# isgasho/h2o-kubernetes

Measured on AMD Instinct MI355X. Metric: GBM train rows/sec on HIGGS-shape 11M×28 at 1/2/4/8 MI355X; AUC parity, higher is better.
Workload: dtype fp32 gradients/hessians; histograms in fixed-point int32 (stochastic rounding) summed exactly in int64; fp64 split gains; exact int64 leaf sums; uint8 bins; 1 GPU; model=GBM bernoulli, global_batch=11000000, rows_per_gpu=11000000, cols=28, max_depth=5, nbins=255, parallelism=dp1

## Files before the change

### h2omx/csrc/tree_kernels.hip

```cpp
#include "common.h"
#include "p2p_device.h"
#include <math.h>

#include <algorithm>
#include <cstdlib>

namespace {

struct SplitParams {
  int mode;
  int leaf_mode;
  int F;
  int is_last_level;
  double min_rows;
  double min_child_weight;
  double lambda_;
  double alpha;
  double gamma;
  double min_split_improvement;
  double learn_rate;
  double max_abs_leaf;
  uint32_t seed;
  int tree_index;
  int depth;
// ... 643 lines not shown
      if (2 * ks > lv.max_next_nodes) ks = lv.max_next_nodes / 2;
      *res_s = ks;
    }
  }
  __syncthreads();
  return *res_s;
}

struct LevelFin {
  LevelOut lv;
  int* ticket;
};

template <int MODE>
__device__ void level_fin_records(const FeatBest* __restrict__ fbest, const int* __restrict__ ctl, const SplitParams& p,
                                  int nbt, const LevelOut& lv) {
  const int n = ctl[CTL_N];
  const int lane = threadIdx.x & 63, wid = threadIdx.x >> 6, nw = blockDim.x >> 6;
  for (int node = wid; node < n; node += nw) node_best_wave<MODE>(fbest, p.F, node, lane, lv.nsplit);
  __syncthreads();
  level_finalize_body(ctl, p, nbt, lv);
}

constexpr int CMP_STAGE_BYTES = 2048;
constexpr int HB_PF = 1;

template <int NBT, int ROWS, int PKM, bool ROUTE, bool CMP, int COP = 1, bool NID16 = false>
__global__ __launch_bounds__(1024) void hist_build_kernel(
    const uint8_t* __restrict__ codes, int64_t npad, const float* __restrict__ g, const float* __restrict__ s2,
    const int* __restrict__ nid, const NodeLink* __restrict__ link, const int* __restrict__ ctl,
    const int* __restrict__ nvb, const double* __restrict__ qscale, uint32_t salt, int F, int fg, int n_groups,
    int wgpg, int slot_lo, int slot_cnt, const short* __restrict__ slot16, unsigned long long* __restrict__ pk_buf,
    unsigned long long* __restrict__ partials, const PartInfo* __restrict__ part_prev,
    const int* __restrict__ ctl_prev, int* __restrict__ nid_out, int writer, GradFuse gf, LevelPro lp,
    const uint8_t* __restrict__ joint, const int* __restrict__ plane_src) {
  salt = (uint32_t)qscale[9];
  extern __shared__ __attribute__((aligned(16))) unsigned long long lds64[];
  __shared__ int width_s[256], rep_s[256];
  __shared__ float rcp_s[256];
  __shared__ NodeSplit pro_ns[ROUTE ? PRO_MAX_NODES : 1];
  __shared__ PartInfo pro_ps[ROUTE ? PRO_MAX_NODES : 1];
  __shared__ int pro_res;
  bool pro = false;
  if constexpr (ROUTE) pro = lp.fbest != nullptr;
  int n_slots;
  if (pro) n_slots = level_prologue(lp, ctl_prev, NBT, blockIdx.x == 0 && writer != 0, pro_ns, pro_ps, &pro_res);
  else n_slots = ctl[CTL_SLOTS];
  const int b = blockIdx.x;
  const int xcd = b & 7, i = b >> 3;
  const int group = i % n_groups;
  const int chunk = xcd + 8 * (i / n_groups);
  const bool route_w = ROUTE && writer && group == 0 && ctl_prev[CTL_N] > 0;
  const bool build = slot_lo < n_slots;
  if (!build && !route_w) return;
  const int f0 = group * fg;
  const int nf = min(fg, F - f0);
  static_assert(COP == 1 || ((PKM == 1 || PKM == 3 || PKM == 6) && !ROUTE && !CMP), "copies: level-0 kernel only");
  const int hist_elems = slot_cnt * fg * NBT;
// ... 2 lines not shown
    const int sp = plane_src ? plane_src[f0 + fi] : f0 + fi;
    return sp >= 0 ? codes + (int64_t)sp * npad : joint + (int64_t)(~sp) * npad;
  };

  for (int j = threadIdx.x; j < hist_elems * COP; j += blockDim.x) lds64[j] = 0ull;
  if (threadIdx.x < fg) {
    const int fi = threadIdx.x;
    const int w = (fi < nf) ? nvb[f0 + fi] + 1 : NBT;
    width_s[fi] = w;
    int r = NBT / w;
    r = r < 1 ? 1 : (r > 64 ? 64 : r);
    if (COP > 1) r = 1;
    rep_s[fi] = r;
    rcp_s[fi] = 1.0f / (float)r;
  }
  __shared__ float tval_s[PKM == 5 ? GF_LDS_NODES : 1];
  if constexpr (PKM == 5) {
    if (gf.apply && gf.cap <= GF_LDS_NODES)
      for (int j = threadIdx.x; j < gf.cap; j += blockDim.x) tval_s[j] = gf.tree[j].value;
  }
  const float sg = (float)qscale[0], ss = (float)qscale[1];
  const int64_t rb = (int64_t)qscale[7];
  const int64_t n_rows = (int64_t)qscale[8];
  __syncthreads();

  const int64_t units = npad / ROWS;
  const int64_t u0 = units * chunk / wgpg, u1 = units * (chunk + 1) / wgpg;
  const int64_t ustart = CMP ? u0 + (threadIdx.x & ~63) : u0 + threadIdx.x;
  for (int64_t uu = ustart; uu < u1; uu += blockDim.x) {
    const bool inb = !CMP || uu + lane < u1;
    const int64_t u = CMP ? (inb ? uu + lane : u1 - 1) : uu;
    const int64_t r0 = u * ROWS;
    int s[ROWS];
    bool any = false;
    if constexpr (ROUTE) {
      int nn[ROWS], nx[ROWS];
      if (nid == nullptr) {
#pragma unroll
        for (int k = 0; k < ROWS; ++k) nn[k] = (r0 + k < n_rows) ? 0 : INT32_MIN;
      } else if constexpr (NID16) {
        const short* n16 = reinterpret_cast<const short*>(nid);
#pragma unroll
        for (int q = 0; q < ROWS / 8; ++q) {
          const uint4 v = *reinterpret_cast<const uint4*>(n16 + r0 + 8 * q);
          const uint32_t w4[4] = {v.x, v.y, v.z, v.w};
#pragma unroll
          for (int k = 0; k < 8; ++k) nn[8 * q + k] = (int)(short)(w4[k >> 1] >> (16 * (k & 1)));
        }
      } else {
#pragma unroll
        for (int q = 0; q < ROWS / 4; ++q) {
          const int4 n4 = *reinterpret_cast<const int4*>(nid + r0 + 4 * q);
          nn[4 * q] = n4.x; nn[4 * q + 1] = n4.y; nn[4 * q + 2] = n4.z; nn[4 * q + 3] = n4.w;
        }
      }
#pragma unroll
      for (int k = 0; k < ROWS; ++k) { nx[k] = nn[k]; s[k] = -1; }
      const int n_prev = pro ? min(ctl_prev[CTL_N], PRO_MAX_NODES) : ctl_prev[CTL_N];
      for (int j = 0; j < n_prev; ++j) {
        bool mine = false;
#pragma unroll
        for (int k = 0; k < ROWS; ++k) mine |= (nn[k] == j);
        if (!mine) continue;
        const PartInfo pj = pro ? pro_ps[j] : part_prev[j];
        if (pj.child < 0) {
#pragma unroll
          for (int k = 0; k < ROWS; ++k)
            if (nn[k] == j) nx[k] = ~pj.gid;
          continue;
        }
        uint32_t cw[ROWS / 4];
        const uint8_t* cp = codes + (int64_t)pj.feat * npad + r0;
        if constexpr (ROWS == 16) {
          const uint4 c4 = *reinterpret_cast<const uint4*>(cp);
          cw[0] = c4.x; cw[1] = c4.y; cw[2] = c4.z; cw[3] = c4.w;
        } else {
          const uint2 c2 = *reinterpret_cast<const uint2*>(cp);
          cw[0] = c2.x; cw[1] = c2.y;
        }
        const int sl_l = (int)(short)(pj.pad & 0xFFFF), sl_r = pj.pad >> 16;
#pragma unroll
        for (int k = 0; k < ROWS; ++k) {
          if (nn[k] == j) {
            const int bc = (cw[k >> 2] >> (8 * (k & 3))) & 0xff;
            const int right = part_right(pj, bc, NBT);
            nx[k] = pj.child + right;
            s[k] = right ? sl_r : sl_l;
          }
        }
      }
#pragma unroll
      for (int k = 0; k < ROWS; ++k) {
        int sl = s[k] - slot_lo;
        if (sl < 0 || sl >= slot_cnt || !build) sl = -1;
        s[k] = sl;
        any |= (sl >= 0);
      }
      if (route_w) {
        if constexpr (NID16) {
          short* o16 = reinterpret_cast<short*>(nid_out);
#pragma unroll
// ... 1074 lines not shown

constexpr int PART_LDS_NODES = 256;

__device__ __forceinline__ int leaf_reps(const double* __restrict__ qs) {
  const int r = (int)qs[10];
  return r < 1 ? 1 : r;
}
constexpr int LEAF_REPS_MAX = 16;
__device__ __forceinline__ long long leaf_sum(const unsigned long long* __restrict__ acc, int64_t i, int reps,
                                              int64_t stride) {
  unsigned long long x[LEAF_REPS_MAX];
#pragma unroll
  for (int r = 0; r < LEAF_REPS_MAX; ++r) x[r] = r < reps ? acc[i + r * stride] : 0ull;
  long long v = 0;
#pragma unroll
  for (int r = 0; r < LEAF_REPS_MAX; ++r) v += (long long)x[r];
  for (int r = LEAF_REPS_MAX; r < reps; ++r) v += (long long)acc[i + r * stride];
  return v;
}
__device__ __forceinline__ void leaf_zero(unsigned long long* __restrict__ acc, int64_t i, int reps, int64_t stride) {
  for (int r = 0; r < reps; ++r) acc[i + r * stride] = 0ull;
}

template <bool PREF, int RPL, int NIDM = 0>
__global__ __launch_bounds__(256) void partition_kernel(const uint8_t* __restrict__ codes, int64_t npad,
                                                        int* nid, const PartInfo* __restrict__ part,
                                                        int nbt, const float* __restrict__ g,
                                                        const float* __restrict__ h, const float* __restrict__ w,
                                                        const double* __restrict__ qs, int cap,
                                                        unsigned long long* __restrict__ leaf_acc,
                                                        const int* __restrict__ ctl_cur,
                                                        const int* __restrict__ ctl_next, int win_max, int R,
                                                        short* __restrict__ slot16, int* nid_out, int all_rows,
                                                        const float* __restrict__ Fm, const float* __restrict__ yv,
                                                        GradParams gp, const uint8_t* __restrict__ y8,
                                                        LevelPro lp) {
  extern __shared__ __attribute__((aligned(16))) unsigned long long lacc[];
  __shared__ PartInfo ps[PART_LDS_NODES];
  __shared__ NodeSplit pro_ns[PRO_MAX_NODES];
  __shared__ int pro_res;
  const bool pro = lp.fbest != nullptr;
  int n_next = 0;
  if (pro) n_next = 2 * level_prologue(lp, ctl_cur, nbt, blockIdx.x == 0, pro_ns, ps, &pro_res);
  const bool use_lds = leaf_acc != nullptr && win_max > 0;
  const int base = all_rows ? 0 : ctl_cur[CTL_BASE];
  const int win = use_lds ? (all_rows ? win_max : min(win_max, ctl_cur[CTL_N] + (pro ? n_next : ctl_next[CTL_N]))) : 0;
  const int n_cur = ctl_cur[CTL_N];
  const bool rec_lds = pro || n_cur <= PART_LDS_NODES;
  if (rec_lds && !pro)
    for (int j = threadIdx.x; j < n_cur; j += blockDim.x) ps[j] = part[j];
  if (use_lds)
    for (int j = threadIdx.x; j < 3 * win * R; j += blockDim.x) lacc[j] = 0ull;
  __syncthreads();
  const int copy = (threadIdx.x & 63) % R;
  float lg = 0, lh = 0, lw = 0;
  if (leaf_acc) { lg = (float)qs[4]; lh = (float)qs[5]; lw = (float)qs[6]; }
  const int64_t nq = npad / RPL;
  for (int64_t q = (int64_t)blockIdx.x * blockDim.x + threadIdx.x; q < nq; q += (int64_t)gridDim.x * blockDim.x) {
    const int64_t r0 = q * RPL;
    int nn[RPL];
    if constexpr (NIDM & 1) {
      static_assert(RPL % 8 == 0, "int16 node ids: 8-row vectors");
#pragma unroll
      for (int v = 0; v < RPL / 8; ++v) {
        const uint4 q4 = *reinterpret_cast<const uint4*>(reinterpret_cast<const short*>(nid) + r0 + 8 * v);
        const uint32_t w4[4] = {q4.x, q4.y, q4.z, q4.w};
#pragma unroll
        for (int k = 0; k < 8; ++k) nn[8 * v + k] = (int)(short)(w4[k >> 1] >> (16 * (k & 1)));
      }
    } else {
#pragma unroll
      for (int v = 0; v < RPL / 4; ++v) {
        const int4 na = *reinterpret_cast<int4*>(nid + r0 + 4 * v);
        nn[4 * v] = na.x; nn[4 * v + 1] = na.y; nn[4 * v + 2] = na.z; nn[4 * v + 3] = na.w;
      }
    }
    float gv[RPL], hv[RPL], wv8[RPL];
    if (PREF) {
#pragma unroll
      for (int v = 0; v < RPL / 4; ++v) {
        if (Fm != nullptr) {
          const float4 f0 = *reinterpret_cast<const float4*>(Fm + r0 + 4 * v);
          float4 y0;
          if (y8 != nullptr) {
            const uint32_t b4 = *reinterpret_cast<const uint32_t*>(y8 + r0 + 4 * v);
            y0 = make_float4((float)(b4 & 0xff), (float)((b4 >> 8) & 0xff), (float)((b4 >> 16) & 0xff),
                             (float)(b4 >> 24));
          } else {
            y0 = *reinterpret_cast<const float4*>(yv + r0 + 4 * v);
          }
          const float fa[4] = {f0.x, f0.y, f0.z, f0.w}, ya[4] = {y0.x, y0.y, y0.z, y0.w};
#pragma unroll
          for (int k = 0; k < 4; ++k) dist_grad(gp.dist, fa[k], ya[k], gp, gv[4 * v + k], hv[4 * v + k]);
        } else {
          const float4 g0 = *reinterpret_cast<const float4*>(g + r0 + 4 * v);
          const float4 h0 = *reinterpret_cast<const float4*>(h + r0 + 4 * v);
          gv[4 * v] = g0.x; gv[4 * v + 1] = g0.y; gv[4 * v + 2] = g0.z; gv[4 * v + 3] = g0.w;
          hv[4 * v] = h0.x; hv[4 * v + 1] = h0.y; hv[4 * v + 2] = h0.z; hv[4 * v + 3] = h0.w;
        }
        if (w) {
          const float4 w0 = *reinterpret_cast<const float4*>(w + r0 + 4 * v);
          wv8[4 * v] = w0.x; wv8[4 * v + 1] = w0.y; wv8[4 * v + 2] = w0.z; wv8[4 * v + 3] = w0.w;
        } else {
          wv8[4 * v] = wv8[4 * v + 1] = wv8[4 * v + 2] = wv8[4 * v + 3] = 1.0f;
        }
      }
    }
    bool changed = false;
    int sv[RPL];
    {
      PartInfo pi[RPL];
      int bc[RPL];
#pragma unroll
      for (int k = 0; k < RPL; ++k) {
        const int n = nn[k] >= 0 ? nn[k] : 0;
        pi[k] = rec_lds ? ps[n] : part[n];
      }
#pragma unroll
      for (int k = 0; k < RPL; ++k) {
        const int f = (nn[k] >= 0 && pi[k].child >= 0) ? pi[k].feat : 0;
        bc[k] = codes[(int64_t)f * npad + r0 + k];
      }
#pragma unroll
      for (int k = 0; k < RPL; ++k) {
        sv[k] = -1;
        const int n = nn[k];
        int leaf = -1;
        if (n < 0) {
          if (!all_rows) continue;
          leaf = ~n;
        } else {
          changed = true;
          const PartInfo& p = pi[k];
          if (p.child < 0) {
            leaf = p.gid;
          } else {
            const int b = bc[k];
            const int right = part_right(p, b, nbt);
            if (p.leaf_children) {
              leaf = p.child_gid + right;
            } else {
              nn[k] = p.child + right;
              sv[k] = right ? (p.pad >> 16) : (int)(short)(p.pad & 0xFFFF);
            }
// ... 617 lines not shown
  return copy_level_out(lp.lv, level_out);
}

static int hist_build_launch(const uint8_t* codes, int64_t npad, const float* g, const float* s2, const int* nid,
                             const void* link, const int* ctl, const int* nvb, const double* qscale, int salt,
                             int F, int nbt, int fg, int n_groups, int wgpg, int slot_lo, int slot_cnt,
                             int rows_per_lane, int threads, const short* slot16, unsigned long long* pk_buf,
                             int pkm, unsigned long long* partials, const void* part_prev, const int* ctl_prev,
                             int* nid_out, int writer, hipStream_t stream, const GradFuse* gfp = nullptr,
                             const LevelPro* lpp = nullptr, const uint8_t* joint = nullptr,
                             const int* plane_src = nullptr) {
  if ((joint == nullptr) != (plane_src == nullptr)) return kBadArg;
  const bool route = part_prev != nullptr;
  GradFuse gfz{};
  if (gfp) gfz = *gfp;
  LevelPro lpz{};
  if (lpp) lpz = *lpp;
  if (lpp && (!route || !writer || lpz.fbest == nullptr || lpz.lv.nsplit == nullptr || lpz.lv.ctl_next != ctl ||
              (const void*)lpz.lv.part != part_prev))
    return kBadArg;
  const bool cmp = (pkm & 8) != 0;
  const int cop = (pkm & 16) ? 8 : ((pkm & 32) ? 4 : 1);
  const bool nid16 = (pkm & 64) != 0;
  pkm &= 7;
  if (nid16 && (!route || cmp || rows_per_lane != 16)) return kBadArg;
  if (cop > 1 && ((pkm != 1 && pkm != 3 && pkm != 6) || route || cmp)) return kBadArg;
  if (pkm == 6 && (nid != nullptr || route || cmp || pk_buf == nullptr)) return kBadArg;
  if (cmp && ((pkm != 2 && pkm != 4) || rows_per_lane != 16 || slot_cnt > 64)) return kBadArg;
  if (route && (ctl_prev == nullptr || nid_out == nullptr || nid_out == nid || (pkm != 2 && pkm != 4)))
    return kBadArg;
  const PartInfo* pp = reinterpret_cast<const PartInfo*>(part_prev);
  if (wgpg % 8 != 0 || npad % 16 != 0 || fg > 256 || threads % 64 != 0 || threads > 1024 || threads < fg)
    return kBadArg;
  if (pkm < 0 || pkm > 6 || (pkm > 0 && pk_buf == nullptr) || ((pkm == 2 || pkm == 4) && !route && slot16 == nullptr))
    return kBadArg;
  if ((pkm == 5) != (gfp != nullptr) || (pkm == 5 && (nid != nullptr || route || cmp || gfz.F == nullptr ||
                                                      gfz.y == nullptr || gfz.g == nullptr || gfz.h == nullptr ||
                                                      (gfz.apply && (gfz.nid == nullptr || gfz.tree == nullptr)))))
    return kBadArg;
  const int64_t units = npad / rows_per_lane;
  if ((units + wgpg - 1) / wgpg * rows_per_lane > ROWS_CAP) return kBadArg;
  const size_t lds = (size_t)slot_cnt * fg * nbt * cop * sizeof(unsigned long long) +
                     (cmp ? (size_t)(threads / 64) * CMP_STAGE_BYTES : 0);
  if (lds > 156 * 1024) return kBadArg;
  const int grid = n_groups * wgpg;
  const NodeLink* lk = reinterpret_cast<const NodeLink*>(link);
#define LAUNCH_HBK(NB, R, M, RT, C)                                                                           \
  hipLaunchKernelGGL((hist_build_kernel<NB, R, M, RT, C>), dim3(grid), dim3(threads), lds, stream, codes, npad, \
                     g, s2, nid, lk, ctl, nvb, qscale, (uint32_t)salt, F, fg, n_groups, wgpg, slot_lo, slot_cnt,  \
                     slot16, pk_buf, partials, pp, ctl_prev, nid_out, writer, gfz, lpz, joint, plane_src)
#define LAUNCH_HBKC(NB, R, M, CP)                                                                                \
  hipLaunchKernelGGL((hist_build_kernel<NB, R, M, false, false, CP>), dim3(grid), dim3(threads), lds, stream, codes, \
                     npad, g, s2, nid, lk, ctl, nvb, qscale, (uint32_t)salt, F, fg, n_groups, wgpg, slot_lo,        \
                     slot_cnt, slot16, pk_buf, partials, pp, ctl_prev, nid_out, writer, gfz, lpz, joint, plane_src)
#define LAUNCH_HBK16(NB, M)                                                                                      \
  hipLaunchKernelGGL((hist_build_kernel<NB, 16, M, true, false, 1, true>), dim3(grid), dim3(threads), lds, stream, \
                     codes, npad, g, s2, nid, lk, ctl, nvb, qscale, (uint32_t)salt, F, fg, n_groups, wgpg, slot_lo,    \
                     slot_cnt, slot16, pk_buf, partials, pp, ctl_prev, nid_out, writer, gfz, lpz, joint, plane_src)
#define LAUNCH_HB(NB, R)                                            \
  do {                                                             \
    if (pkm == 0) LAUNCH_HBK(NB, R, 0, false, false);               \
    else if (pkm == 1 && cop == 8) LAUNCH_HBKC(NB, R, 1, 8);        \
    else if (pkm == 3 && cop == 8) LAUNCH_HBKC(NB, R, 3, 8);        \
    else if (pkm == 1 && cop == 4) LAUNCH_HBKC(NB, R, 1, 4);        \
    else if (pkm == 3 && cop == 4) LAUNCH_HBKC(NB, R, 3, 4);        \
    else if (pkm == 6 && cop == 8) LAUNCH_HBKC(NB, R, 6, 8);        \
    else if (pkm == 6 && cop == 4) LAUNCH_HBKC(NB, R, 6, 4);        \
    else if (pkm == 6) LAUNCH_HBK(NB, R, 6, false, false);          \
    else if (pkm == 1) LAUNCH_HBK(NB, R, 1, false, false);          \
    else if (pkm == 2 && route) LAUNCH_HBK(NB, R, 2, true, false);  \
    else if (pkm == 2) LAUNCH_HBK(NB, R, 2, false, false);          \
    else if (pkm == 3) LAUNCH_HBK(NB, R, 3, false, false);          \
    else if (pkm == 5) LAUNCH_HBK(NB, R, 5, false, false);          \
    else if (route) LAUNCH_HBK(NB, R, 4, true, false);              \
    else LAUNCH_HBK(NB, R, 4, false, false);                        \
  } while (0)
#define LAUNCH_HBCMP(NB)                                             \
  do {                                                              \
    if (pkm == 2 && route) LAUNCH_HBK(NB, 16, 2, true, true);        \
    else if (pkm == 2) LAUNCH_HBK(NB, 16, 2, false, true);           \
    else if (route) LAUNCH_HBK(NB, 16, 4, true, true);               \
// ... 258 lines not shown
  const p2pdev::P2PDesc d = *reinterpret_cast<const p2pdev::P2PDesc*>(desc);
  if (d.world < 2 || d.world > p2pdev::kMaxRanks || d.rank < 0 || d.rank >= d.world) return kBadArg;
  const SplitParams p = *reinterpret_cast<const SplitParams*>(params);
  LevelOut lv{};
  if (!copy_level_out(lv, level_out)) return kBadArg;
  hipLaunchKernelGGL(node_best_finalize_p2p_kernel, dim3(1), dim3(1024), 0, stream, d, ctl, p, nbt, lv);
  return launch_status();
}

constexpr int PARTITION_BLOCKS = 8192;
constexpr int PART_RPL = 8;

static int partition_launch(const uint8_t* codes, int64_t npad, int* nid, const void* part, int nbt, const float* g,
                            const float* h, const float* w, const double* qscale, int cap,
                            unsigned long long* leaf_acc, const int* ctl_cur, const int* ctl_next, int win_max,
                            int blocks, int prefetch, short* slot16, int* nid_out, int all_rows, hipStream_t stream,
                            const float* Fm = nullptr, const float* yv = nullptr, const GradParams* gpp = nullptr,
                            int nidm = 0, const uint8_t* y8 = nullptr, const LevelPro* lpp = nullptr) {
  LevelPro lpz{};
  if (lpp) lpz = *lpp;
  if (lpp && (lpz.fbest == nullptr || lpz.lv.nsplit == nullptr || lpz.lv.ctl_next != ctl_next ||
              (const void*)lpz.lv.part != part))
    return kBadArg;
  if (nidm != 0 && nid_out == nid) return kBadArg;
  GradParams gp{};
  if (gpp) gp = *gpp;
  if ((Fm != nullptr) != (gpp != nullptr) || (Fm != nullptr && (yv == nullptr || w != nullptr || !prefetch)))
    return kBadArg;
  if (slot16 && prefetch) return kBadArg;
  if (npad % PART_RPL != 0 || blocks < 1 || blocks > PARTITION_BLOCKS || win_max < 0) return kBadArg;
  if (all_rows && (leaf_acc == nullptr || win_max > cap)) return kBadArg;
  constexpr size_t kWinLds = 64 * 1024;
  int R = 8;
  while (R > 1 && (size_t)3 * win_max * R * sizeof(unsigned long long) > kWinLds) R >>= 1;
  if ((size_t)3 * win_max * R * sizeof(unsigned long long) > kWinLds) {
    if (all_rows) return kBadArg;
    win_max = 0;
  }
  const size_t lds = (leaf_acc && win_max > 0) ? (size_t)3 * win_max * R * sizeof(unsigned long long) : 0;
#define LAUNCH_PK(PF, NM, WIN)                                                                                  \
  hipLaunchKernelGGL((partition_kernel<PF, PART_RPL, NM>), dim3(blocks), dim3(256), lds, stream, codes, npad, nid, \
                     reinterpret_cast<const PartInfo*>(part), nbt, g, h, w, qscale, cap, leaf_acc, ctl_cur,        \
                     ctl_next, WIN, R, slot16, nid_out, all_rows, Fm, yv, gp, y8, lpz)
  if (prefetch && leaf_acc) {
    if (nidm == 3) LAUNCH_PK(true, 3, win_max);
    else if (nidm & 1) LAUNCH_PK(true, 1, win_max);
    else LAUNCH_PK(true, 0, win_max);
  } else {
    if (nidm == 3) LAUNCH_PK(false, 3, leaf_acc ? win_max : 0);
    else if (nidm == 1) LAUNCH_PK(false, 1, leaf_acc ? win_max : 0);
    else if (nidm == 2) LAUNCH_PK(false, 2, leaf_acc ? win_max : 0);
    else LAUNCH_PK(false, 0, leaf_acc ? win_max : 0);
  }
#undef LAUNCH_PK
  return launch_status();
}

H2OMX_API int h2omx_partition(const uint8_t* codes, int64_t npad, int* nid, const void* part, int nbt, const float* g,
                              const float* h, const float* w, const double* qscale, int cap,
                              unsigned long long* leaf_acc, const int* ctl_cur, const int* ctl_next, int win_max,
                              int blocks, int prefetch, short* slot16, hipStream_t stream) {
  return partition_launch(codes, npad, nid, part, nbt, g, h, w, qscale, cap, leaf_acc, ctl_cur, ctl_next, win_max,
                          blocks, prefetch, slot16, nid, 0, stream);
}

H2OMX_API int h2omx_partition_route(const uint8_t* codes, int64_t npad, const int* nid_in, int* nid_out,
                                    const void* part, int nbt, const int* ctl_cur, const int* ctl_next, int blocks,
                                    short* slot16, int nidm, hipStream_t stream) {
  if (slot16 == nullptr) return kBadArg;
  return partition_launch(codes, npad, const_cast<int*>(nid_in), part, nbt, nullptr, nullptr, nullptr, nullptr, 0,
                          nullptr, ctl_cur, ctl_next, 0, blocks, 0, slot16, nid_out, 0, stream, nullptr, nullptr,
                          nullptr, nidm);
}

H2OMX_API int h2omx_partition_final(const uint8_t* codes, int64_t npad, const int* nid_in, int* nid_out,
                                    const void* part, int nbt, const float* g, const float* h, const float* w,
                                    const double* qscale, int cap, unsigned long long* leaf_acc, const int* ctl_cur,
                                    const int* ctl_next, int blocks, const float* Fm, const float* y,
                                    const void* gparams, int nidm, const uint8_t* y8, hipStream_t stream) {
  return partition_launch(codes, npad, const_cast<int*>(nid_in), part, nbt, g, h, w, qscale, cap, leaf_acc, ctl_cur,
                          ctl_next, cap, blocks, 1, nullptr, nid_out, 1, stream, Fm, y,
                          reinterpret_cast<const GradParams*>(gparams), nidm, y8);
}

H2OMX_API int h2omx_partition_route_fin(const uint8_t* codes, int64_t npad, const int* nid_in, int* nid_out, void* part,
                                        int nbt, const int* ctl_cur, int* ctl_next, int blocks, short* slot16,
                                        int nidm, const void* fbest, const void* params, const void* level_out,
// ... 2261 lines not shown
```

### h2omx/models/tree/engine.py

```python
from __future__ import annotations

import ctypes
import math
import os
from dataclasses import dataclass, field

import numpy as np
import torch

from ... import ops
from .binning import BinnedMatrix
from ...utils.trace import PhaseTimer
from .structs import (FEAT_BEST_BYTES, NODE_LINK_BYTES, NODE_SPLIT_BYTES, PART_INFO_BYTES, TREE_NODE_DTYPE, GradParams,
                      LevelOut, SplitParams, check_layout, interaction_masks)


@dataclass
class TreeParams:
    max_depth: int = 5
    min_rows: float = 10.0
    min_child_weight: float = 0.0
    reg_lambda: float = 0.0
    reg_alpha: float = 0.0
    gamma: float = 0.0
# ... 25 lines not shown
    THREADS = 1024
    TARGET_WGS = 512
    ROWS_PER_LANE = 16
    ROWS_CAP = 262144
    SYNC_NODE_CAP = 4096
    SEG_TARGET_CHUNKS = 1024
    SEG_LDS_BUDGET = 16 * 1024
    SEG_LDS_BUDGET_WIDE = 64 * 1024
    SCAN_SLOTS = 1
    MEAN_LEAVES_NO_H = True
    BAG_COMPACT = True
    bag_compact = False
    DEEP_DEPTH = 10
    FUSE_MAX_DEPTH = 8
    FUSE_MAX_PREV = 4
    CLOSE_SINGLE_BLOCK = 2048
    DIRECT_MIN_NODES = 2048
    DIRECT_MAX_ELIG = 32.0
    DIRECT_WAVE_ROWS = 512
    PART_WAVE_NODES = 2048
    DIRECT_CHUNKED = True
    PART_BLOCKS = 1024
    FUSE_ROUTE = True
    BUNDLE = True
    PK32 = True
    FUSE_GRAD = False
    CHAIN_BEGIN = True
    LEAF_REPS = 16
    FUSE_FIN = True
    FUSE_FIN_LOCAL = False
    FIN_PROLOGUE = True
    FIN_PROLOGUE_FINAL = False
    PERMUTE_GS = True
    ECODES = True
    LF_MULTI_BLOCK = True
    COLMAJOR_EVERY = 0

    def __init__(self, bm: BinnedMatrix, params: TreeParams, comm=None):
        if not bm.codes.is_cuda:
            raise ValueError("HipTreeBuilder needs device-resident codes")
        self.lib = ops.tree_lib()
        check_layout(self.lib)
        self.bm = bm
        self.p = params
        self.comm = comm
        self.dev = bm.codes.device
# ... 251 lines not shown
        F, nbt = self.F, self.nbt
        Fh, nvb_h, joint, plane_src, feat_plane = self._hist_planes()
        spp = self._params(tree_index)
        sp = self._sp
        comm = self.comm if (self.comm is not None and self.comm.world_size > 1) else None
        p2p = getattr(comm, "p2p", None) if comm is not None else None

        if comm is not None and stat is None:
            comm.all_reduce_(smax, "max")
        s2 = w if p.mode == 0 else h
        link = [self._buf("link0", 4, torch.int32), None]
        T = self.timer.phase
        if not chain:
            with T("tree_begin"):
                self.begin(smax, tree_index)
        pk_boost = chain and self.pk_in_boost
        full_prev = None
        max_depth = p.max_depth
        final_ctl = self.ctl[max_depth % 2]
        max_nodes = 1
        fuse = self.fuse_route
        nid16 = self.nid16 is not None
        nid_buf = self.nid16 if nid16 else (self.nid, self.nid2)
        part_prev = None
        pend = None
        for d in range(max_depth):
            cur, nxt = d % 2, (d + 1) % 2
            ctl_cur, ctl_nxt = self.ctl[cur], self.ctl[nxt]
            if max_nodes > self.SYNC_NODE_CAP:
                n_now, s_now = [int(v) for v in ctl_cur[:2].tolist()]
                self.stats["host_syncs"] += 1
                if n_now == 0:
                    final_ctl = ctl_cur
                    break
                max_nodes, max_slots = n_now, s_now
            else:
                max_slots = 1 if d == 0 else max(1, max_nodes // 2)
            last = d == max_depth - 1
            plan = self.plan_level(max_slots)
            l0_copies = d == 0 and grad_fuse is None and self.L0_COPIES in (4, 8)
            if l0_copies:
                plan = self.plan_l0()
            built = self._buf("built", max_slots * self.per_node, torch.int64)
            full_cur = None if last else self._buf(f"full{cur}", max_nodes * self.per_node, torch.int64)
            sp.depth = d
            sp.children_leaves = 1 if last else 0
# ... 45 lines not shown
                                                         P(self.qscale), spp, nbt, P(fbest), ctypes.addressof(lvo),
                                                         P(self._fin_ticket), P(feat_plane), st),
                              "reduce_split_fin")
                elif rs:
                    ops.check(lib.h2omx_reduce_split(P(partials), wgpg, fg, slot_lo, slot_cnt, P(full_prev),
                                                     P(full_cur), P(ctl_cur), P(link[cur]), P(bm.nvb),
                                                     P(tree_fmask), P(self.qscale), spp, nbt, P(fbest),
                                                     P(feat_plane), st),
                              "reduce_split")
                else:
                    ops.check(lib.h2omx_hist_reduce(P(partials), n_groups, wgpg, fg, F, nbt, slot_lo, slot_cnt,
                                                    P(ctl_cur), P(built), st), "hist_reduce")
            hist_elems = plan["slot_cnt"] * plan["fg"] * nbt
            partials = self._buf("partials", plan["n_groups"] * plan["wgpg"] * hist_elems, torch.int64)
            for ps in range(plan["passes"]):
                slot_lo = ps * plan["slot_cnt"]
                with T("hist"):
                    if d > 0 and pend is not None:
                        ops.check(lib.h2omx_hist_build_route_fin(
                            P(bm.codes), bm.npad, P(None if (d == 1 and self.implicit_root) else nid_buf[(d - 1) % 2]),
                            P(part_prev), P(ctl_nxt), P(nid_buf[d % 2]), P(ctl_cur), P(nvb_h), P(self.qscale),
                            Fh, nbt, plan["fg"], plan["n_groups"], plan["wgpg"], plan["slot_cnt"],
                            self.ROWS_PER_LANE, plan["threads"], P(self.pk),
                            (4 if self.pk32 else 2) + (64 if nid16 else 0), P(partials), *pend["args"],
                            P(joint), P(plane_src), st),
                            "hist_build_route_fin")
                        pend = None
                    elif d > 0 and fuse and self._fused_level(d):
                        ops.check(lib.h2omx_hist_build_route(
                            P(bm.codes), bm.npad, P(None if (d == 1 and self.implicit_root) else nid_buf[(d - 1) % 2]),
                            P(part_prev), P(ctl_nxt),
                            P(nid_buf[d % 2]), 1 if ps == 0 else 0, P(ctl_cur), P(nvb_h), P(self.qscale), Fh, nbt,
                            plan["fg"], plan["n_groups"], plan["wgpg"], slot_lo, plan["slot_cnt"],
                            self.ROWS_PER_LANE, plan["threads"], P(self.pk),
                            (4 if self.pk32 else 2) + (64 if nid16 else 0),
                            P(partials), P(joint), P(plane_src), st),
                            "hist_build_route")
                    elif d == 0 and grad_fuse is not None:
                        gf = grad_fuse
                        ops.check(lib.h2omx_hist_build_grad(
                            P(bm.codes), bm.npad, P(ctl_cur), P(nvb_h), P(self.qscale), tree_index & 0x7FFFFFFF,
                            Fh, nbt, plan["fg"], plan["n_groups"], plan["wgpg"], plan["slot_cnt"],
                            self.ROWS_PER_LANE, plan["threads"], P(self.pk), P(partials), P(gf["F"]), P(gf["y"]),
                            P(self.nid), P(self.tree_buf), self.capacity, P(g), P(h), 1 if gf["apply"] else 0,
                            0 if p.mode == 0 else 1, 0 if self.pk32 else 1, ctypes.addressof(gf["gp"]),
                            P(joint), P(plane_src), st),
                            "hist_build_grad")
                    else:
                        ops.check(lib.h2omx_hist_build(
                            P(bm.codes), bm.npad, P(g), P(s2),
                            P(None if (d == 0 and self.implicit_root) else (nid_buf[d % 2] if fuse else self.nid)),
                            P(link[cur]), P(ctl_cur), P(nvb_h),
                            P(self.qscale), tree_index & 0x7FFFFFFF, Fh, nbt, plan["fg"], plan["n_groups"],
                            plan["wgpg"], slot_lo, plan["slot_cnt"], self.ROWS_PER_LANE, plan["threads"],
                            P(self.slot16), P(self.pk),
                            ((6 if pk_boost else 1 + (2 if self.pk32 else 0)) if d == 0
                             else 2 + (2 if self.pk32 else 0))
                            + ({8: 16, 4: 32}.get(self.L0_COPIES, 0) if l0_copies else 0),
# ... 15 lines not shown
                    spc = type(sp).from_buffer_copy(sp)
                    pro_args = (P(fbest), ctypes.addressof(spc), ctypes.addressof(lvo), max_nodes)
                    if pro == "hist":
                        pend = dict(args=pro_args, keep=(spc, lvo, fbest, nl, nsplit, self._bufs.get("fbcat")))
                elif fuse_p2p:
                    ops.check(lib.h2omx_node_best_finalize_p2p(p2p.desc_ptr, P(ctl_cur), spp, nbt,
                                                               ctypes.addressof(lvo), st), "node_best_finalize_p2p")
                else:
                    ops.check(lib.h2omx_level_finalize(P(fbest), P(ctl_cur), spp, nbt, ctypes.addressof(lvo),
                                                       max_nodes, self._lf_tiles(max_nodes), st), "level_finalize")
            win = min(3 * max_nodes, self.capacity)
            with T("partition"):
                if fuse and last:
                    rg = self.regrad if (chain and w is None) else None
                    leaf16 = chain and nid16
                    self.leaf16_buf = nid_buf[(d + 1) % 2] if leaf16 else None
                    pf_args = (P(bm.codes), bm.npad, P(nid_buf[d % 2]),
                               P(self.leaf16_buf if leaf16 else self.nid),
                               P(part), nbt, P(g), P(h), P(w), P(self.qscale),
                               self.capacity, P(self.leaf_acc), P(ctl_cur), P(ctl_nxt),
                               self.part_blocks, P(rg[0] if rg else None),
                               P(rg[1] if rg else None),
                               ctypes.addressof(rg[2]) if rg else None,
                               (3 if leaf16 else 1) if nid16 else 0,
                               P(rg[3] if rg else None))
                    if pro == "final":
                        ops.check(lib.h2omx_partition_final_fin(*pf_args, *pro_args, st),
                                  "partition_final_fin")
                    else:
                        ops.check(lib.h2omx_partition_final(*pf_args, st), "partition_final")
                elif fuse and not self._fused_level(d + 1):
                    pr_args = (P(bm.codes), bm.npad, P(nid_buf[d % 2]), P(nid_buf[(d + 1) % 2]), P(part), nbt,
                               P(ctl_cur), P(ctl_nxt), self.part_blocks, P(self.slot16), 3 if nid16 else 0)
                    if pro == "route":
                        ops.check(lib.h2omx_partition_route_fin(*pr_args, *pro_args, st),
                                  "partition_route_fin")
                    else:
                        ops.check(lib.h2omx_partition_route(*pr_args, st), "partition_route")
                elif not fuse:
                    ops.check(lib.h2omx_partition(P(bm.codes), bm.npad, P(self.nid), P(part), nbt, P(g), P(h),
                                                  P(w), P(self.qscale), self.capacity, P(self.leaf_acc),
                                                  P(ctl_cur), P(ctl_nxt), win, self.part_blocks, 1 if last else 0,
                                                  P(None if last else self.slot16), st),
                              "partition")
            part_prev = part
            full_prev = full_cur
            max_nodes = next_nodes
        leaf_p2p = p2p is not None and self.gbound is None and self.capacity * 3 * 8 * p2p.world <= p2p.cap
        if comm is not None and not leaf_p2p:
            with T("allreduce"):
                comm.all_reduce_(self.leaf_acc)
        with T("leaf"):
            if leaf_p2p:
                ops.check(lib.h2omx_leaf_finalize_p2p(p2p.desc_ptr, P(self.leaf_acc), P(final_ctl), P(self.qscale),
                                                      spp, P(self.tree_buf), self.capacity, 1 if chain else 0,
                                                      P(smax if chain else None), p.mode,
                                                      self.max_rows_per_wg if chain else 0,
                                                      P(self.ctl[0] if chain else None),
                                                      P(link[0] if chain else None), self.row_base,
                                                      P(self.tree_ctr if chain else None), st), "leaf_finalize_p2p")
                comm.stats["p2p_calls"] += 1
                comm.stats["p2p_bytes"] += self.capacity * 3 * 8
            elif chain:
                ops.check(lib.h2omx_leaf_finalize_begin(P(self.leaf_acc), P(final_ctl), P(self.qscale), spp,
                                                        P(self.tree_buf), self.capacity, P(smax), p.mode,
# ... 392 lines not shown
```

### h2omx/ops/__init__.py

```python
from __future__ import annotations

import ctypes

from .. import _native

_CT = {"P": ctypes.c_void_p, "I": ctypes.c_int, "L": ctypes.c_int64, "F": ctypes.c_float,
       "D": ctypes.c_double, "S": ctypes.c_void_p, "U": ctypes.c_uint32}

TREE_SIGS = {
    "h2omx_tree_sizes": "P",
    "h2omx_bin_features": "PLLIPPIPLS",
    "h2omx_hist_build": "PLPPPPPPPIIIIIIIIIIPPIPPPS",
    "h2omx_hist_reduce": "PIIIIIIIPPS",
    "h2omx_hist_build_route": "PLPPPPIPPPIIIIIIIIIPIPPPS",
    "h2omx_hist_build_grad": "PLPPPIIIIIIIIIPPPPPPIPPIIIPPPS",
    "h2omx_split_find": "PPPPPPPPPIIPS",
    "h2omx_reduce_split": "PIIIIPPPPPPPPIPPS",
    "h2omx_reduce_split_p2p": "PPIIIPPPPPPPPIIPS",
    "h2omx_reduce_split_fin": "PIIIPPPPPPPPIPPPPS",
    "h2omx_bundle_plane": "PLLIPIPS",
    "h2omx_node_best_finalize_p2p": "PPPIPS",
    "h2omx_leaf_finalize_p2p": "PPPPPPIIPIIPPLPS",
    "h2omx_level_finalize": "PPPIPIPS",
    "h2omx_partition": "PLPPIPPPPIPPPIIIPS",
    "h2omx_partition_blocks": "",
    "h2omx_partition_final": "PLPPPIPPPPIPPPIPPPIPS",
    "h2omx_partition_route": "PLPPPIPPIPIS",
    "h2omx_hist_build_route_fin": "PLPPPPPPPIIIIIIIIPIPPPPIPPS",
    "h2omx_partition_route_fin": "PLPPPIPPIPIPPPIS",
    "h2omx_partition_final_fin": "PLPPPIPPPPIPPPIPPPIPPPPIS",
    "h2omx_leaf_reduce": "PIIPS",
    "h2omx_boost_update": "PPPLLPPPPPPPLPIPIPPIIPPS",
    "h2omx_apply_tree": "PLPPS",
    "h2omx_tree_archive": "PLPIPS",
    "h2omx_sketch_bins": "",
    "h2omx_sketch": "PLIIIPIPPPPPPPPPPPPS",
    "h2omx_softmax_grad": "PILPPLLIPPPPPPS",
    "h2omx_oob_accumulate": "PPLPPPUIFLIS",
    "h2omx_stat_blocks": "",
    "h2omx_stat_reduce": "PPS",
    "h2omx_tree_begin": "PIIPPPPILIPS",
    "h2omx_leaf_stats": "PPPPLPIPS",
    "h2omx_leaf_finalize": "PPPPPIS",
    "h2omx_leaf_finalize_begin": "PPPPPIPIIPPLPS",
    "h2omx_leaf_finalize_mono": "PPPPPIPS",
    "h2omx_predict_raw": "PLLPPIIPLPS",
    "h2omx_predict_binned": "PLLPPIIIPLPS",
    "h2omx_pc_rows": "",
    "h2omx_tree_begin_seg": "PIIPPPPIPIIIPPPPPLIPS",
    "h2omx_bag_compact": "PLPPPPPPPPPIS",
# ... 135 lines not shown
```

Before: 16.17 billion rows/s (row-trees per second, all GPUs).

## Route rows by feature list: preload distinct split-feature code planes per unit

Builds a per-level list of the distinct split features (up to 8) among the previous level's nodes using wave ballots. Each lane then loads those features' code bytes for its row unit up front and selects among them with register selects, instead of issuing a dependent gather per node inside the node loop. By default this is enabled only in the fused hist-build routing path, with the partition kernels gated behind flags. The cost is more register pressure from the cv arrays, extra loads when only some features are needed, and LDS setup per block.

```diff
diff --git a/h2omx/csrc/tree_kernels.hip b/h2omx/csrc/tree_kernels.hip
--- a/h2omx/csrc/tree_kernels.hip
+++ b/h2omx/csrc/tree_kernels.hip
@@ -689,6 +689,62 @@
   level_finalize_body(ctl, p, nbt, lv);
 }
 
+constexpr int ROUTE_MAX_FEATS = 8;
+constexpr int ROUTE_LIST_NODES = 64;
+struct RouteList {
+  int d_f;
+  int flist[ROUTE_LIST_NODES];
+  int fidx[ROUTE_LIST_NODES];
+};
+
+__device__ __forceinline__ void route_feat_list(const PartInfo* ps, int n, RouteList* rl) {
+  const int lane = threadIdx.x & 63;
+  bool live = false;
+  int f = -1;
+  if (lane < n) {
+    live = ps[lane].child >= 0;
+    f = ps[lane].feat;
+  }
+  unsigned long long rem = __ballot(live);
+  int d = 0, idx = 0;
+  while (rem != 0ull) {
+    const int lead = __ffsll((long long)rem) - 1;
+    const int fl = __builtin_amdgcn_readlane(f, lead);
+    const bool m = live && f == fl;
+    if (m) idx = d;
+    if (lane == 0) rl->flist[d] = fl;
+    rem &= ~__ballot(m);
+    ++d;
+  }
+  if (lane < n) rl->fidx[lane] = idx;
+  if (lane == 0) rl->d_f = d;
+}
+
+template <int ROWS>
+__device__ __forceinline__ void load_row_codes(const uint8_t* cp, uint32_t* cw) {
+  static_assert(ROWS == 8 || ROWS == 16, "8- or 16-row units");
+  if constexpr (ROWS == 16) {
+    const uint4 c4 = *reinterpret_cast<const uint4*>(cp);
+    cw[0] = c4.x; cw[1] = c4.y; cw[2] = c4.z; cw[3] = c4.w;
+  } else {
+    const uint2 c2 = *reinterpret_cast<const uint2*>(cp);
+    cw[0] = c2.x; cw[1] = c2.y;
+  }
+}
+
+__global__ __launch_bounds__(64) void route_feat_list_kernel(const PartInfo* __restrict__ part, int n,
+                                                             int* __restrict__ out) {
+  __shared__ PartInfo ps[ROUTE_LIST_NODES];
+  __shared__ RouteList rl;
+  for (int j = threadIdx.x; j < n; j += blockDim.x) ps[j] = part[j];
+  __syncthreads();
+  route_feat_list(ps, n, &rl);
+  __syncthreads();
+  if (threadIdx.x == 0) out[0] = rl.d_f;
+  if ((int)threadIdx.x < rl.d_f) out[1 + threadIdx.x] = rl.flist[threadIdx.x];
+  if ((int)threadIdx.x < n) out[1 + ROUTE_LIST_NODES + threadIdx.x] = rl.fidx[threadIdx.x];
+}
+
 constexpr int CMP_STAGE_BYTES = 2048;
 constexpr int HB_PF = 1;
 
@@ -700,7 +756,7 @@
     int wgpg, int slot_lo, int slot_cnt, const short* __restrict__ slot16, unsigned long long* __restrict__ pk_buf,
     unsigned long long* __restrict__ partials, const PartInfo* __restrict__ part_prev,
     const int* __restrict__ ctl_prev, int* __restrict__ nid_out, int writer, GradFuse gf, LevelPro lp,
-    const uint8_t* __restrict__ joint, const int* __restrict__ plane_src) {
+    const uint8_t* __restrict__ joint, const int* __restrict__ plane_src, int route_bf) {
   salt = (uint32_t)qscale[9];
   extern __shared__ __attribute__((aligned(16))) unsigned long long lds64[];
   __shared__ int width_s[256], rep_s[256];
@@ -749,7 +805,28 @@
   const float sg = (float)qscale[0], ss = (float)qscale[1];
   const int64_t rb = (int64_t)qscale[7];
   const int64_t n_rows = (int64_t)qscale[8];
+  __shared__ int rl_raw[ROUTE ? sizeof(RouteList) / sizeof(int) : 1];
+  RouteList* rl = reinterpret_cast<RouteList*>(rl_raw);
+  int d_f = -1;
+  bool list = false;
+  if constexpr (ROUTE) {
+    list = route_bf != 0 && ctl_prev[CTL_N] <= ROUTE_LIST_NODES;
+    if (list && !pro)
+      for (int j = threadIdx.x; j < ctl_prev[CTL_N]; j += blockDim.x) pro_ps[j] = part_prev[j];
+  }
   __syncthreads();
+  const uint8_t* rplane[ROUTE ? ROUTE_MAX_FEATS : 1];
+  if constexpr (ROUTE) {
+    if (list) {
+      if (threadIdx.x < 64) route_feat_list(pro_ps, ctl_prev[CTL_N], rl);
+      __syncthreads();
+      d_f = __builtin_amdgcn_readfirstlane(rl->d_f);
+      if (d_f > ROUTE_MAX_FEATS) d_f = -1;
+#pragma unroll
+      for (int j = 0; j < ROUTE_MAX_FEATS; ++j)
+        rplane[j] = codes + (int64_t)__builtin_amdgcn_readfirstlane(j < d_f ? rl->flist[j] : 0) * npad;
+    }
+  }
 
   const int64_t units = npad / ROWS;
   const int64_t u0 = units * chunk / wgpg, u1 = units * (chunk + 1) / wgpg;
@@ -762,6 +839,15 @@
     bool any = false;
     if constexpr (ROUTE) {
       int nn[ROWS], nx[ROWS];
+      uint32_t cv[ROUTE_MAX_FEATS][ROWS / 4];
+      if (d_f >= 0) {
+#pragma unroll
+        for (int j = 0; j < ROUTE_MAX_FEATS; ++j) {
+#pragma unroll
+          for (int q = 0; q < ROWS / 4; ++q) cv[j][q] = 0u;
+          if (j < d_f) load_row_codes<ROWS>(rplane[j] + r0, cv[j]);
+        }
+      }
       if (nid == nullptr) {
 #pragma unroll
         for (int k = 0; k < ROWS; ++k) nn[k] = (r0 + k < n_rows) ? 0 : INT32_MIN;
@@ -789,7 +875,7 @@
 #pragma unroll
         for (int k = 0; k < ROWS; ++k) mine |= (nn[k] == j);
         if (!mine) continue;
-        const PartInfo pj = pro ? pro_ps[j] : part_prev[j];
+        const PartInfo pj = (pro || list) ? pro_ps[j] : part_prev[j];
         if (pj.child < 0) {
 #pragma unroll
           for (int k = 0; k < ROWS; ++k)
@@ -797,13 +883,24 @@
           continue;
         }
         uint32_t cw[ROWS / 4];
-        const uint8_t* cp = codes + (int64_t)pj.feat * npad + r0;
-        if constexpr (ROWS == 16) {
-          const uint4 c4 = *reinterpret_cast<const uint4*>(cp);
-          cw[0] = c4.x; cw[1] = c4.y; cw[2] = c4.z; cw[3] = c4.w;
+        if (d_f >= 0) {
+          const int fi = rl->fidx[j];
+#pragma unroll
+          for (int q = 0; q < ROWS / 4; ++q) cw[q] = cv[0][q];
+#pragma unroll
+          for (int jj = 1; jj < ROUTE_MAX_FEATS; ++jj) {
+#pragma unroll
+            for (int q = 0; q < ROWS / 4; ++q) cw[q] = fi == jj ? cv[jj][q] : cw[q];
+          }
         } else {
-          const uint2 c2 = *reinterpret_cast<const uint2*>(cp);
-          cw[0] = c2.x; cw[1] = c2.y;
+          const uint8_t* cp = codes + (int64_t)pj.feat * npad + r0;
+          if constexpr (ROWS == 16) {
+            const uint4 c4 = *reinterpret_cast<const uint4*>(cp);
+            cw[0] = c4.x; cw[1] = c4.y; cw[2] = c4.z; cw[3] = c4.w;
+          } else {
+            const uint2 c2 = *reinterpret_cast<const uint2*>(cp);
+            cw[0] = c2.x; cw[1] = c2.y;
+          }
         }
         const int sl_l = (int)(short)(pj.pad & 0xFFFF), sl_r = pj.pad >> 16;
 #pragma unroll
@@ -1924,7 +2021,7 @@
   for (int r = 0; r < reps; ++r) acc[i + r * stride] = 0ull;
 }
 
-template <bool PREF, int RPL, int NIDM = 0>
+template <bool PREF, int RPL, int NIDM = 0, bool BYF = false>
 __global__ __launch_bounds__(256) void partition_kernel(const uint8_t* __restrict__ codes, int64_t npad,
                                                         int* nid, const PartInfo* __restrict__ part,
                                                         int nbt, const float* __restrict__ g,
@@ -1939,6 +2036,8 @@
                                                         LevelPro lp) {
   extern __shared__ __attribute__((aligned(16))) unsigned long long lacc[];
   __shared__ PartInfo ps[PART_LDS_NODES];
+  __shared__ int rl_raw[BYF ? sizeof(RouteList) / sizeof(int) : 1];
+  RouteList& rl = *reinterpret_cast<RouteList*>(rl_raw);
   __shared__ NodeSplit pro_ns[PRO_MAX_NODES];
   __shared__ int pro_res;
   const bool pro = lp.fbest != nullptr;
@@ -1954,6 +2053,17 @@
   if (use_lds)
     for (int j = threadIdx.x; j < 3 * win * R; j += blockDim.x) lacc[j] = 0ull;
   __syncthreads();
+  int d_f = -1;
+  const uint8_t* rplane[ROUTE_MAX_FEATS];
+  if (BYF && rec_lds && n_cur <= ROUTE_LIST_NODES) {
+    if (threadIdx.x < 64) route_feat_list(ps, n_cur, &rl);
+    __syncthreads();
+    d_f = __builtin_amdgcn_readfirstlane(rl.d_f);
+    if (d_f > ROUTE_MAX_FEATS) d_f = -1;
+#pragma unroll
+    for (int j = 0; j < ROUTE_MAX_FEATS; ++j)
+      rplane[j] = codes + (int64_t)__builtin_amdgcn_readfirstlane(j < d_f ? rl.flist[j] : 0) * npad;
+  }
   const int copy = (threadIdx.x & 63) % R;
   float lg = 0, lh = 0, lw = 0;
   if (leaf_acc) { lg = (float)qs[4]; lh = (float)qs[5]; lw = (float)qs[6]; }
@@ -1975,6 +2085,15 @@
       for (int v = 0; v < RPL / 4; ++v) {
         const int4 na = *reinterpret_cast<int4*>(nid + r0 + 4 * v);
         nn[4 * v] = na.x; nn[4 * v + 1] = na.y; nn[4 * v + 2] = na.z; nn[4 * v + 3] = na.w;
+      }
+    }
+    uint32_t cv[ROUTE_MAX_FEATS][RPL / 4];
+    if (BYF && d_f >= 0) {
+#pragma unroll
+      for (int j = 0; j < ROUTE_MAX_FEATS; ++j) {
+#pragma unroll
+        for (int v = 0; v < RPL / 4; ++v) cv[j][v] = 0u;
+        if (j < d_f) load_row_codes<RPL>(rplane[j] + r0, cv[j]);
       }
     }
     float gv[RPL], hv[RPL], wv8[RPL];
@@ -2018,10 +2137,23 @@
         const int n = nn[k] >= 0 ? nn[k] : 0;
         pi[k] = rec_lds ? ps[n] : part[n];
       }
-#pragma unroll
-      for (int k = 0; k < RPL; ++k) {
-        const int f = (nn[k] >= 0 && pi[k].child >= 0) ? pi[k].feat : 0;
-        bc[k] = codes[(int64_t)f * npad + r0 + k];
+      if (BYF && d_f >= 0) {
+        int fi[RPL];
+#pragma unroll
+        for (int k = 0; k < RPL; ++k) fi[k] = rl.fidx[nn[k] >= 0 ? nn[k] : 0];
+#pragma unroll
+        for (int k = 0; k < RPL; ++k) {
+          uint32_t cw = cv[0][k >> 2];
+#pragma unroll
+          for (int j = 1; j < ROUTE_MAX_FEATS; ++j) cw = fi[k] == j ? cv[j][k >> 2] : cw;
+          bc[k] = (cw >> (8 * (k & 3))) & 0xff;
+        }
+      } else {
+#pragma unroll
+        for (int k = 0; k < RPL; ++k) {
+          const int f = (nn[k] >= 0 && pi[k].child >= 0) ? pi[k].feat : 0;
+          bc[k] = codes[(int64_t)f * npad + r0 + k];
+        }
       }
 #pragma unroll
       for (int k = 0; k < RPL; ++k) {
@@ -2685,7 +2817,9 @@
   const bool cmp = (pkm & 8) != 0;
   const int cop = (pkm & 16) ? 8 : ((pkm & 32) ? 4 : 1);
   const bool nid16 = (pkm & 64) != 0;
+  const int rbf = (pkm & 128) != 0 ? 1 : 0;
   pkm &= 7;
+  if (rbf && !route) return kBadArg;
   if (nid16 && (!route || cmp || rows_per_lane != 16)) return kBadArg;
   if (cop > 1 && ((pkm != 1 && pkm != 3 && pkm != 6) || route || cmp)) return kBadArg;
   if (pkm == 6 && (nid != nullptr || route || cmp || pk_buf == nullptr)) return kBadArg;
@@ -2711,15 +2845,15 @@
 #define LAUNCH_HBK(NB, R, M, RT, C)                                                                           \
   hipLaunchKernelGGL((hist_build_kernel<NB, R, M, RT, C>), dim3(grid), dim3(threads), lds, stream, codes, npad, \
                      g, s2, nid, lk, ctl, nvb, qscale, (uint32_t)salt, F, fg, n_groups, wgpg, slot_lo, slot_cnt,  \
-                     slot16, pk_buf, partials, pp, ctl_prev, nid_out, writer, gfz, lpz, joint, plane_src)
+                     slot16, pk_buf, partials, pp, ctl_prev, nid_out, writer, gfz, lpz, joint, plane_src, rbf)
 #define LAUNCH_HBKC(NB, R, M, CP)                                                                                \
   hipLaunchKernelGGL((hist_build_kernel<NB, R, M, false, false, CP>), dim3(grid), dim3(threads), lds, stream, codes, \
                      npad, g, s2, nid, lk, ctl, nvb, qscale, (uint32_t)salt, F, fg, n_groups, wgpg, slot_lo,        \
-                     slot_cnt, slot16, pk_buf, partials, pp, ctl_prev, nid_out, writer, gfz, lpz, joint, plane_src)
+                     slot_cnt, slot16, pk_buf, partials, pp, ctl_prev, nid_out, writer, gfz, lpz, joint, plane_src, rbf)
 #define LAUNCH_HBK16(NB, M)                                                                                      \
   hipLaunchKernelGGL((hist_build_kernel<NB, 16, M, true, false, 1, true>), dim3(grid), dim3(threads), lds, stream, \
                      codes, npad, g, s2, nid, lk, ctl, nvb, qscale, (uint32_t)salt, F, fg, n_groups, wgpg, slot_lo,    \
-                     slot_cnt, slot16, pk_buf, partials, pp, ctl_prev, nid_out, writer, gfz, lpz, joint, plane_src)
+                     slot_cnt, slot16, pk_buf, partials, pp, ctl_prev, nid_out, writer, gfz, lpz, joint, plane_src, rbf)
 #define LAUNCH_HB(NB, R)                                            \
   do {                                                             \
     if (pkm == 0) LAUNCH_HBK(NB, R, 0, false, false);               \
@@ -3024,6 +3158,8 @@
   if (lpp && (lpz.fbest == nullptr || lpz.lv.nsplit == nullptr || lpz.lv.ctl_next != ctl_next ||
               (const void*)lpz.lv.part != part))
     return kBadArg;
+  const int rbf = (nidm >> 2) & 1;
+  nidm &= 3;
   if (nidm != 0 && nid_out == nid) return kBadArg;
   GradParams gp{};
   if (gpp) gp = *gpp;
@@ -3040,10 +3176,15 @@
     win_max = 0;
   }
   const size_t lds = (leaf_acc && win_max > 0) ? (size_t)3 * win_max * R * sizeof(unsigned long long) : 0;
-#define LAUNCH_PK(PF, NM, WIN)                                                                                  \
-  hipLaunchKernelGGL((partition_kernel<PF, PART_RPL, NM>), dim3(blocks), dim3(256), lds, stream, codes, npad, nid, \
-                     reinterpret_cast<const PartInfo*>(part), nbt, g, h, w, qscale, cap, leaf_acc, ctl_cur,        \
+#define LAUNCH_PKB(PF, NM, WIN, BF)                                                                             \
+  hipLaunchKernelGGL((partition_kernel<PF, PART_RPL, NM, BF>), dim3(blocks), dim3(256), lds, stream, codes, npad, \
+                     nid, reinterpret_cast<const PartInfo*>(part), nbt, g, h, w, qscale, cap, leaf_acc, ctl_cur,  \
                      ctl_next, WIN, R, slot16, nid_out, all_rows, Fm, yv, gp, y8, lpz)
+#define LAUNCH_PK(PF, NM, WIN)            \
+  do {                                    \
+    if (rbf) LAUNCH_PKB(PF, NM, WIN, true); \
+    else LAUNCH_PKB(PF, NM, WIN, false);  \
+  } while (0)
   if (prefetch && leaf_acc) {
     if (nidm == 3) LAUNCH_PK(true, 3, win_max);
     else if (nidm & 1) LAUNCH_PK(true, 1, win_max);
@@ -3055,6 +3196,7 @@
     else LAUNCH_PK(false, 0, leaf_acc ? win_max : 0);
   }
 #undef LAUNCH_PK
+#undef LAUNCH_PKB
   return launch_status();
 }
 
@@ -3063,8 +3205,17 @@
                               unsigned long long* leaf_acc, const int* ctl_cur, const int* ctl_next, int win_max,
                               int blocks, int prefetch, short* slot16, hipStream_t stream) {
   return partition_launch(codes, npad, nid, part, nbt, g, h, w, qscale, cap, leaf_acc, ctl_cur, ctl_next, win_max,
-                          blocks, prefetch, slot16, nid, 0, stream);
-}
+                          blocks, prefetch & 1, slot16, nid, 0, stream, nullptr, nullptr, nullptr,
+                          (prefetch & 2) ? 4 : 0);
+}
+
+H2OMX_API int h2omx_route_feat_list(const void* part, int n, int* out, hipStream_t stream) {
+  if (part == nullptr || out == nullptr || n < 0 || n > ROUTE_LIST_NODES) return kBadArg;
+  hipLaunchKernelGGL(route_feat_list_kernel, dim3(1), dim3(64), 0, stream, reinterpret_cast<const PartInfo*>(part), n,
+                     out);
+  return launch_status();
+}
+H2OMX_API int h2omx_route_max_feats() { return ROUTE_MAX_FEATS; }
 
 H2OMX_API int h2omx_partition_route(const uint8_t* codes, int64_t npad, const int* nid_in, int* nid_out,
                                     const void* part, int nbt, const int* ctl_cur, const int* ctl_next, int blocks,
diff --git a/h2omx/models/tree/engine.py b/h2omx/models/tree/engine.py
--- a/h2omx/models/tree/engine.py
+++ b/h2omx/models/tree/engine.py
@@ -71,6 +71,8 @@
     DIRECT_CHUNKED = True
     PART_BLOCKS = 1024
     FUSE_ROUTE = True
+    ROUTE_BY_FEATURE = True
+    ROUTE_BY_FEATURE_SITES = ("hist",)
     BUNDLE = True
     PK32 = True
     FUSE_GRAD = False
@@ -368,6 +370,9 @@
         fuse = self.fuse_route
         nid16 = self.nid16 is not None
         nid_buf = self.nid16 if nid16 else (self.nid, self.nid2)
+        sites = self.ROUTE_BY_FEATURE_SITES if self.ROUTE_BY_FEATURE else ()
+        rbf_h, rbf_r, rbf_p = (128 if "hist" in sites else 0, 4 if "route" in sites else 0,
+                               4 if "final" in sites else 0)
         part_prev = None
         pend = None
         for d in range(max_depth):
@@ -459,7 +464,7 @@
                             P(part_prev), P(ctl_nxt), P(nid_buf[d % 2]), P(ctl_cur), P(nvb_h), P(self.qscale),
                             Fh, nbt, plan["fg"], plan["n_groups"], plan["wgpg"], plan["slot_cnt"],
                             self.ROWS_PER_LANE, plan["threads"], P(self.pk),
-                            (4 if self.pk32 else 2) + (64 if nid16 else 0), P(partials), *pend["args"],
+                            (4 if self.pk32 else 2) + (64 if nid16 else 0) + rbf_h, P(partials), *pend["args"],
                             P(joint), P(plane_src), st),
                             "hist_build_route_fin")
                         pend = None
@@ -470,7 +475,7 @@
                             P(nid_buf[d % 2]), 1 if ps == 0 else 0, P(ctl_cur), P(nvb_h), P(self.qscale), Fh, nbt,
                             plan["fg"], plan["n_groups"], plan["wgpg"], slot_lo, plan["slot_cnt"],
                             self.ROWS_PER_LANE, plan["threads"], P(self.pk),
-                            (4 if self.pk32 else 2) + (64 if nid16 else 0),
+                            (4 if self.pk32 else 2) + (64 if nid16 else 0) + rbf_h,
                             P(partials), P(joint), P(plane_src), st),
                             "hist_build_route")
                     elif d == 0 and grad_fuse is not None:
@@ -532,7 +537,7 @@
                                self.part_blocks, P(rg[0] if rg else None),
                                P(rg[1] if rg else None),
                                ctypes.addressof(rg[2]) if rg else None,
-                               (3 if leaf16 else 1) if nid16 else 0,
+                               ((3 if leaf16 else 1) if nid16 else 0) + rbf_p,
                                P(rg[3] if rg else None))
                     if pro == "final":
                         ops.check(lib.h2omx_partition_final_fin(*pf_args, *pro_args, st),
@@ -541,7 +546,7 @@
                         ops.check(lib.h2omx_partition_final(*pf_args, st), "partition_final")
                 elif fuse and not self._fused_level(d + 1):
                     pr_args = (P(bm.codes), bm.npad, P(nid_buf[d % 2]), P(nid_buf[(d + 1) % 2]), P(part), nbt,
-                               P(ctl_cur), P(ctl_nxt), self.part_blocks, P(self.slot16), 3 if nid16 else 0)
+                               P(ctl_cur), P(ctl_nxt), self.part_blocks, P(self.slot16), (3 if nid16 else 0) + rbf_r)
                     if pro == "route":
                         ops.check(lib.h2omx_partition_route_fin(*pr_args, *pro_args, st),
                                   "partition_route_fin")
@@ -550,7 +555,8 @@
                 elif not fuse:
                     ops.check(lib.h2omx_partition(P(bm.codes), bm.npad, P(self.nid), P(part), nbt, P(g), P(h),
                                                   P(w), P(self.qscale), self.capacity, P(self.leaf_acc),
-                                                  P(ctl_cur), P(ctl_nxt), win, self.part_blocks, 1 if last else 0,
+                                                  P(ctl_cur), P(ctl_nxt), win, self.part_blocks,
+                                                  (1 if last else 0) + rbf_p // 2,
                                                   P(None if last else self.slot16), st),
                               "partition")
             part_prev = part
diff --git a/h2omx/ops/__init__.py b/h2omx/ops/__init__.py
--- a/h2omx/ops/__init__.py
+++ b/h2omx/ops/__init__.py
@@ -26,6 +26,8 @@
     "h2omx_partition_blocks": "",
     "h2omx_partition_final": "PLPPPIPPPPIPPPIPPPIPS",
     "h2omx_partition_route": "PLPPPIPPIPIS",
+    "h2omx_route_feat_list": "PIPS",
+    "h2omx_route_max_feats": "",
     "h2omx_hist_build_route_fin": "PLPPPPPPPIIIIIIIIPIPPPPIPPS",
     "h2omx_partition_route_fin": "PLPPPIPPIPIPPPIS",
     "h2omx_partition_final_fin": "PLPPPIPPPPIPPPIPPPIPPPPIS",
```

Result: no change. 16.31 billion rows/s (row-trees per second, all GPUs) (median of 6 runs) (+0.8%).
